# ferreiraluisa/implementation-phd-lab-vision

Hardware: AMD Instinct MI355X
Metric: H36M frames/sec ResNet-50 feature extraction (higher is better)
Workload: dtype bf16; 1 GPU; ResNet-50[:-1] bf16 forward, batch 256 x 224x224x3 fp32 NCHW frames per GPU (BASELINE configs[1]), seeded synthetic weights, (N,2048) fp32 features; batch_per_gpu=256, micro_batch=0, lanes=2, lanes_requested=2, lanes_mode=2 lanes (1.092 x one lane), input=f32, parallelism=frames sharded over 1 rank(s)

## Files before the change

### implementation_phd_lab_vision_amd/csrc/kernels.h

```cpp
#pragma once
#include <hip/hip_runtime.h>
#include <stdint.h>
#include <type_traits>

typedef __attribute__((ext_vector_type(8))) __bf16 bf16x8;
typedef __attribute__((ext_vector_type(4))) float f32x4;
typedef __attribute__((ext_vector_type(4))) unsigned int u32x4;
typedef __attribute__((ext_vector_type(2))) unsigned int u32x2;

#define GLOBAL_AS __attribute__((address_space(1)))
#define LDS_AS __attribute__((address_space(3)))

__device__ __forceinline__ float bf16_bits_to_f32(unsigned int hi16) { return __uint_as_float(hi16 << 16); }

__device__ __forceinline__ unsigned int pack_bf16x2(float lo, float hi) {
    typedef __attribute__((ext_vector_type(2))) __bf16 bf16x2;
    typedef __attribute__((ext_vector_type(2))) float f32x2;
    f32x2 v = {lo, hi};
    bf16x2 b = __builtin_convertvector(v, bf16x2);
    return __builtin_bit_cast(unsigned int, b);
}

typedef __attribute__((ext_vector_type(8))) _Float16 f16x8;
typedef __attribute__((ext_vector_type(2))) _Float16 f16x2;

template <int ET>
__device__ __forceinline__ f32x4 mfma_e(bf16x8 a, bf16x8 b, f32x4 c) {
    if constexpr (ET == 0) return __builtin_amdgcn_mfma_f32_16x16x32_bf16(a, b, c, 0, 0, 0);
    else return __builtin_amdgcn_mfma_f32_16x16x32_f16(__builtin_bit_cast(f16x8, a), __builtin_bit_cast(f16x8, b), c, 0, 0, 0);
}
typedef __attribute__((ext_vector_type(16))) float f32x16;
template <int ET>
__device__ __forceinline__ f32x16 mfma32_e(bf16x8 a, bf16x8 b, f32x16 c) {
    if constexpr (ET == 0) return __builtin_amdgcn_mfma_f32_32x32x16_bf16(a, b, c, 0, 0, 0);
    else return __builtin_amdgcn_mfma_f32_32x32x16_f16(__builtin_bit_cast(f16x8, a), __builtin_bit_cast(f16x8, b), c, 0, 0, 0);
}
typedef __attribute__((ext_vector_type(8))) int i32x8;
__device__ __forceinline__ f32x4 mfma_fp8_k128(bf16x8 a0, bf16x8 a1, bf16x8 b0, bf16x8 b1, f32x4 c) {
    const u32x4 al = __builtin_bit_cast(u32x4, a0), ah = __builtin_bit_cast(u32x4, a1);
    const u32x4 bl = __builtin_bit_cast(u32x4, b0), bh = __builtin_bit_cast(u32x4, b1);
    const i32x8 a = {(int)al[0], (int)al[1], (int)al[2], (int)al[3], (int)ah[0], (int)ah[1], (int)ah[2], (int)ah[3]};
    const i32x8 b = {(int)bl[0], (int)bl[1], (int)bl[2], (int)bl[3], (int)bh[0], (int)bh[1], (int)bh[2], (int)bh[3]};
    return __builtin_amdgcn_mfma_scale_f32_16x16x128_f8f6f4(a, b, c, 0, 0, 0, 0x7f7f7f7f, 0, 0x7f7f7f7f);
}
__device__ __forceinline__ unsigned pack4_fp8(float v0, float v1, float v2, float v3) {
    v0 = __builtin_amdgcn_fmed3f(v0, -448.0f, 448.0f); v1 = __builtin_amdgcn_fmed3f(v1, -448.0f, 448.0f);
    v2 = __builtin_amdgcn_fmed3f(v2, -448.0f, 448.0f); v3 = __builtin_amdgcn_fmed3f(v3, -448.0f, 448.0f);
    int w = __builtin_amdgcn_cvt_pk_fp8_f32(v0, v1, 0, false);
    w = __builtin_amdgcn_cvt_pk_fp8_f32(v2, v3, w, true);
    return (unsigned)w;
}
template <int ET>
__device__ __forceinline__ unsigned int pack2_e(float lo, float hi) {
    if constexpr (ET == 0) {
        return pack_bf16x2(lo, hi);
    } else {
        lo = __builtin_amdgcn_fmed3f(lo, -65504.0f, 65504.0f);
        hi = __builtin_amdgcn_fmed3f(hi, -65504.0f, 65504.0f);
        const f16x2 b = {(_Float16)lo, (_Float16)hi};
        return __builtin_bit_cast(unsigned int, b);
    }
}
template <int ET>
__device__ __forceinline__ float unpack_lo_e(unsigned int u) {
    if constexpr (ET == 0) return bf16_bits_to_f32(u & 0xffffu);
    else return (float)__builtin_bit_cast(f16x2, u)[0];
}
template <int ET>
__device__ __forceinline__ float unpack_hi_e(unsigned int u) {
    if constexpr (ET == 0) return __uint_as_float(u & 0xffff0000u);
    else return (float)__builtin_bit_cast(f16x2, u)[1];
}

struct FastDiv {
    unsigned mul, shr;
};

struct ConvArgs {
    const __bf16* x;
    const __bf16* w;
    const float* bias;
    const __bf16* res;
    __bf16* y;
    int N, H, W, Cin, Ho, Wo, Cout;
    int ks, stride, pad, relu;
    int M;
    int HoWo;
    int cin_chunks;
    int nk;
    int Ktot;
    int n_ctiles;
    int n_blocks;
    int x_back;
    unsigned x_records;
    unsigned w_bytes;
    unsigned y_bytes;
    FastDiv div_howo, div_wo, div_ctiles;
    int x_cstride;
    int x_wrap;
    int y_cstride;
    int et;
    float oscale, rscale;
    float q_inv;
    const __bf16* x2;
    int H2, W2, stride2, x2_cstride, cc1;
    unsigned x2_records;
#if defined(R50_STAMP)
    unsigned long long* dbg;
#endif
};

#if defined(R50_STAMP)
#define R50_STAMP_DECL unsigned long long st_prev = __builtin_readcyclecounter(), st_sum[8] = {0, 0, 0, 0, 0, 0, 0, 0}; const unsigned long long st_rt0 = __builtin_amdgcn_s_memrealtime();
#define R50_MARK(i) { __builtin_amdgcn_sched_barrier(0); const unsigned long long st_now = __builtin_readcyclecounter(); st_sum[i] += st_now - st_prev; st_prev = st_now; __builtin_amdgcn_sched_barrier(0); }
#define R50_STAMP_FLUSH(nw) st_sum[7] = __builtin_amdgcn_s_memrealtime() - st_rt0;    \
    if (a.dbg && (threadIdx.x & 63) == 0) { _Pragma("unroll") for (int q = 0; q < 8; ++q) \
        a.dbg[((size_t)blockIdx.x * (nw) + (threadIdx.x >> 6)) * 8 + q] = st_sum[q]; }
#else
#define R50_STAMP_DECL
#define R50_MARK(i)
#define R50_STAMP_FLUSH(nw)
#endif

__device__ __forceinline__ unsigned fast_div(unsigned n, FastDiv d) {
    return d.mul == 0u ? n : (__umulhi(n, d.mul) >> d.shr);
}

#ifndef XCD_REMAP
#define XCD_REMAP 1
#endif
__device__ __forceinline__ int xcd_remap(int bid, int nblk) {
    const int q = nblk >> 3, r = nblk & 7, xcd = bid & 7;
    const int base = (xcd < r) ? xcd * (q + 1) : r * (q + 1) + (xcd - r) * q;
    return base + (bid >> 3);
}

template <int LO, int HI>
__device__ __forceinline__ void wait_vmcnt_range(int n) {
    if constexpr (LO == HI) {
        asm volatile("s_waitcnt vmcnt(%0)" ::"n"(LO) : "memory");
    } else {
        constexpr int MID = (LO + HI) / 2;
        if (n <= MID) wait_vmcnt_range<LO, MID>(n);
        else wait_vmcnt_range<MID + 1, HI>(n);
    }
}
__device__ __forceinline__ void wait_vmcnt(int n) { wait_vmcnt_range<0, 63>(n < 0 ? 0 : (n > 63 ? 63 : n)); }

__device__ __forceinline__ unsigned relu_bf16x2(unsigned v) {
    typedef __attribute__((ext_vector_type(2))) short s16x2;
    const s16x2 z = {0, 0};
    return __builtin_bit_cast(unsigned, __builtin_elementwise_max(__builtin_bit_cast(s16x2, v), z));
}

constexpr unsigned kOobOffset = 0x80000000u;

template <int ET, int BC, int BP, int WC, int WP, int NSTAGE, bool SPLIT = false>
__global__ __launch_bounds__(WC * WP * 64) void igemm_bf16_kernel(const ConvArgs a) {
#if defined(__HIP_DEVICE_COMPILE__)
    constexpr int NT = WC * WP * 64;
    constexpr int MR = BC / WC / 16;
    constexpr int NR = BP / WP / 16;
    static_assert(MR >= 2 && (MR % 2) == 0, "wave needs >= 32 couts");
    static_assert(NSTAGE == 2 || NSTAGE == 3, "2 or 3 LDS stages");
    constexpr int RPP = NT / 8;
    static_assert(BC % RPP == 0 && BP % (16 * WP) == 0, "cout rows fill whole staging passes; pixels come in 16-blocks per wave");
    constexpr int WROWS = BC / RPP;
    constexpr int XROWS = (BP + RPP - 1) / RPP;
    constexpr int BP_PAD = XROWS * RPP;
    constexpr int PASS_BYTES = NT * 16;
    constexpr int STAGE_BYTES = (BC + BP_PAD) * 128;
    constexpr int LOADS_PER_STAGE = WROWS + XROWS;
    constexpr int D = NSTAGE - 1;

    extern __shared__ __attribute__((aligned(16))) char smem[];

    const int tid = threadIdx.x;
    const int lane = tid & 63;
    const int wave = __builtin_amdgcn_readfirstlane(tid >> 6);
    const int wave_c = wave / WP, wave_p = wave % WP;
    const int fr = lane & 15, fq = lane >> 4;
    const int srow = tid >> 3;
    const int slot = tid & 7;
    const int lchunk = slot ^ (srow & 7);

    const int grid = gridDim.x;
    const int first = xcd_remap(blockIdx.x, grid);
    const int my_tiles = (a.n_blocks - first + grid - 1) / grid;
    const int total = my_tiles * a.nk;

    const __amdgpu_buffer_rsrc_t rsrc_w =
        __builtin_amdgcn_make_buffer_rsrc(const_cast<__bf16*>(a.w), 0, a.w_bytes, 0x00020000);
    const __amdgpu_buffer_rsrc_t rsrc_x = __builtin_amdgcn_make_buffer_rsrc(
        const_cast<char*>(reinterpret_cast<const char*>(a.x) - a.x_back), 0, a.x_records, 0x00020000);
    const __amdgpu_buffer_rsrc_t rsrc_y = __builtin_amdgcn_make_buffer_rsrc(a.y, 0, a.y_bytes, 0x00020000);
    const __amdgpu_buffer_rsrc_t rsrc_r =
        __builtin_amdgcn_make_buffer_rsrc(const_cast<__bf16*>(a.res), 0, a.res ? a.y_bytes : 0u, 0x00020000);

    unsigned x_voff[XROWS], x_mask[XROWS], w_voff[WROWS];
    auto decode_tile = [&](int tile) {
        const int pt = (int)fast_div((unsigned)tile, a.div_ctiles);
        const int ct = tile - pt * a.n_ctiles;
        const int c0 = ct * BC, p0 = pt * BP;
#pragma unroll
        for (int i = 0; i < XROWS; ++i) {
            const int m = p0 + i * RPP + srow;
            unsigned mask = 0u, voff = kOobOffset;
            if ((BP_PAD == BP || i * RPP + srow < BP) && m < a.M) {
                const int n = (int)fast_div((unsigned)m, a.div_howo);
                const int r = m - n * a.HoWo;
                const int ho = (int)fast_div((unsigned)r, a.div_wo);
                const int wo = r - ho * a.Wo;
                const int hc = ho * a.stride, wc = wo * a.stride;
                voff = (unsigned)(((n * a.H + hc) * a.W + wc) * a.x_cstride + lchunk * 8) * 2u;
                if (a.ks == 1) {
                    mask = 1u;
                } else {
                    const unsigned hm = (hc >= a.pad ? 1u : 0u) | 2u | (hc - a.pad + 2 < a.H ? 4u : 0u);
                    const unsigned wm = (wc >= a.pad ? 1u : 0u) | 2u | (wc - a.pad + 2 < a.W ? 4u : 0u);
                    mask = ((hm & 1u) ? wm : 0u) | ((hm & 2u) ? (wm << 3) : 0u) | ((hm & 4u) ? (wm << 6) : 0u);
                }
            }
            x_voff[i] = voff;
            x_mask[i] = mask;
        }
#pragma unroll
        for (int i = 0; i < WROWS; ++i) {
            const int rho = i * RPP + srow;
            const int cl = (rho & ~31) | (rho & 3) | (((rho >> 4) & 1) << 2) | (((rho >> 2) & 3) << 3);
            w_voff[i] = (unsigned)((c0 + cl) * a.Ktot + lchunk * 8) * 2u;
        }
    };
    int i_tile = first, i_k = 0, i_tap = 0, i_cc = 0, i_dw = 0, i_wofs = 0, i_tapofs = 0, i_buf = 0;
    const int row_adv = (a.W - a.ks) * a.x_cstride * 2;
    decode_tile(i_tile);
    auto stage_issue = [&]() {
        char* sbase = smem + i_buf * STAGE_BYTES;
        const int xcc = (i_cc >= a.x_wrap) ? i_cc - a.x_wrap : i_cc;
        const int xofs = __builtin_amdgcn_readfirstlane(i_tapofs + xcc * 128);
        const int wofs = __builtin_amdgcn_readfirstlane(i_wofs);
        const int tap = __builtin_amdgcn_readfirstlane(i_tap);
#pragma unroll
        for (int i = 0; i < WROWS; ++i)
            __builtin_amdgcn_raw_ptr_buffer_load_lds(rsrc_w, (LDS_AS void*)(sbase + i * PASS_BYTES + wave * 1024), 16,
                                                     w_voff[i], wofs, 0, 0);
#pragma unroll
        for (int i = 0; i < XROWS; ++i) {
            const unsigned voff = ((x_mask[i] >> tap) & 1u) ? x_voff[i] : kOobOffset;
            __builtin_amdgcn_raw_ptr_buffer_load_lds(rsrc_x, (LDS_AS void*)(sbase + BC * 128 + i * PASS_BYTES + wave * 1024),
                                                     16, voff, xofs, 0, 0);
        }
        i_buf = (i_buf == NSTAGE - 1) ? 0 : i_buf + 1;
        i_wofs += 128;
        if (++i_cc == a.cin_chunks) {
            i_cc = 0;
            ++i_tap;
            i_tapofs += a.x_cstride * 2;
            if (++i_dw == a.ks) { i_dw = 0; i_tapofs += row_adv; }
        }
        if (++i_k == a.nk) {
            i_k = 0; i_tap = 0; i_cc = 0; i_dw = 0; i_wofs = 0; i_tapofs = 0;
            i_tile += grid;
            if (i_tile < a.n_blocks) decode_tile(i_tile);
        }
    };

    f32x4 acc[MR][NR];
    constexpr bool BIG = (MR * NR > 16);
    constexpr bool LEAN = (NT >= 1024);
    constexpr bool PREFETCH_RES = !SPLIT && !BIG && !LEAN;
    u32x4 res_reg[PREFETCH_RES ? MR / 2 : 1][PREFETCH_RES ? NR : 1];
    const bool has_res = (a.res != nullptr);
    const int fphys0 = (fq ^ (fr & 7)) << 4;
    const int w_frag = (wave_c * MR * 16 + fr) * 128;
    const int x_frag = BC * 128 + (wave_p * NR * 16 + fr) * 128;
    const int cout_lane = wave_c * MR * 16 + 8 * fq;
    const int pix_lane = wave_p * NR * 16 + fr;
    int c_tile = first, c_k = 0, c_buf = 0;
    unsigned y_voff = 0u;
    const unsigned y_rowstep = (unsigned)(16 * a.y_cstride * 2);

    auto tile_begin = [&]() {
        const int pt = (int)fast_div((unsigned)c_tile, a.div_ctiles);
// ... 2106 lines not shown
                const int prow = (32 * k + srow) % ROWS;
                const int lchunk = (lt & 7) ^ (prow & 7);
                const unsigned p = (unsigned)(p0 + prow);
                const unsigned n = p / HOWO, r = p - n * HOWO, ho = r / OW, wo = r - ho * OW;
                const unsigned q = a.x_sub ? p : (n * WI + 2 * ho) * WI + 2 * wo;
                const bool ok = prow < limit;
                vt[k] = ok ? (p * CT2 + lchunk * 8) * 2u : kOobOffset;
                vx[k] = ok ? (q * CX + lchunk * 8) * 2u : kOobOffset;
            }
        };
        auto issue_x = [&](auto grp_c) {
            constexpr int GRP = decltype(grp_c)::value;
#pragma unroll
            for (int i = 7 * GRP; i < 7 * GRP + 7; ++i) {
                const int sl = __builtin_amdgcn_readfirstlane((32 * i + 8 * w) / ROWS);
                char* dst = smem + XR + i * 4096 + w * 1024;
                if (GRP == 0) __builtin_amdgcn_raw_ptr_buffer_load_lds(rs_t2, (LDS_AS void*)dst, 16, vt[i % 7], sl * 128, 0, 0);
                else __builtin_amdgcn_raw_ptr_buffer_load_lds(rs_x, (LDS_AS void*)dst, 16, vx[i % 7], (sl - 2) * 128, 0, 0);
            }
        };
        using G0 = std::integral_constant<int, 0>;
        using G1 = std::integral_constant<int, 1>;
        using G2 = std::integral_constant<int, 2>;
        f32x4 accB[2][NR];
        unsigned rvo[OC_PASSES];
        auto out_rows = [&](int tile) {
            const int p0 = tile * a.bp;
            const int limit = (a.M - p0 < a.bp) ? a.M - p0 : a.bp;
#pragma unroll
            for (int i = 0; i < OC_PASSES; ++i) {
                const int R = 32 * i + srow;
                const int sl = R / ROWS, prow = R - ROWS * sl;
                const int lchunk = (lt & 7) ^ (prow & 7);
                rvo[i] = (prow < limit) ? (unsigned)((p0 + prow) * COUT + sl * 64 + lchunk * 8) * 2u : kOobOffset;
            }
        };
        auto y1n_store = [&](int tile) {
            const int p0 = tile * a.bp;
            const int limit = (a.M - p0 < a.bp) ? a.M - p0 : a.bp;
#pragma unroll
            for (int j = 0; j < NR; ++j) {
                const f32x4 lo = accB[0][j], hi = accB[1][j];
                u32x4 o = (u32x4){pack2_e<ET>(lo[0], lo[1]), pack2_e<ET>(lo[2], lo[3]), pack2_e<ET>(hi[0], hi[1]), pack2_e<ET>(hi[2], hi[3])};
#pragma unroll
                for (int e = 0; e < 4; ++e) o[e] = relu_bf16x2(o[e]);
                const unsigned voff = (16 * j + fr < limit) ? (unsigned)((p0 + 16 * j + fr) * C1N + 32 * w + 8 * fq) * 2u : kOobOffset;
                __builtin_amdgcn_raw_buffer_store_b128(o, rs_y1, voff, 0, 0);
            }
        };
        auto init_accb = [&]() {
            const f32x4 lo = *reinterpret_cast<const f32x4*>(smem + B1_OFF + (32 * w + 8 * fq) * 4);
            const f32x4 hi = *reinterpret_cast<const f32x4*>(smem + B1_OFF + (32 * w + 8 * fq + 4) * 4);
#pragma unroll
            for (int j = 0; j < NR; ++j) { accB[0][j] = lo; accB[1][j] = hi; }
        };
        x_rows(first);
        issue_x(G0{}); issue_x(G1{}); issue_x(G2{});
        w_load_half(sofs_of(0, 6), wA, 0); w_load_half(sofs_of(0, 6), wA, 1);
        w_load_half(sofs_of(0, 7), wB, 0); w_load_half(sofs_of(0, 7), wB, 1);
        asm volatile("s_waitcnt vmcnt(0) lgkmcnt(0)" ::: "memory");
        __builtin_amdgcn_s_barrier();
        init_accb();
        __builtin_amdgcn_s_barrier();
        unsigned tl = 0;
        R50_STAMP_DECL
        for (int tile = first; tile < a.n_tiles; tile += grid, ++tl) {
            out_rows(tile);
            for (int c = 0; c < NCH; ++c) {
                const char* xb = smem + OUTC + (c & 1) * 2 * SLOT;
                if (c == NCH - 2) x_rows(tile + grid);
                w_step(sofs_of(c + 1, 6), wA, xb, accB[0], accB[1]);
                R50_MARK(2)
                if (c == NCH - 2) { spin_until(0, 4u * (tl + 1)); issue_x(G0{}); }
                R50_MARK(5)
                if (c == NCH - 1) {
                    asm volatile("s_waitcnt vmcnt(4)" ::: "memory");
                    signal(3);
                }
                R50_MARK(6)
                w_step(sofs_of(c + 1, 7), wB, xb + SLOT, accB[0], accB[1]);
                R50_MARK(2)
                if (c == NCH - 2) { spin_until(1, 4u * (tl + 1)); issue_x(G1{}); }
                R50_MARK(5)
#if defined(R50_STAMP)
                __builtin_amdgcn_sched_barrier(0);
                asm volatile("s_nop 0" ::"v"(accB[1][NR - 1]), "v"(accB[0][NR - 1]) : "memory");
#endif
                R50_MARK(2)
                __builtin_amdgcn_sched_barrier(0);
                {
                    const int cofs = __builtin_amdgcn_readfirstlane(c * 256);
                    u32x4 v[OC_PASSES];
#pragma unroll
                    for (int i = 0; i < OC_PASSES; ++i) v[i] = *reinterpret_cast<const u32x4*>(xb + i * 4096 + lt * 16);
#pragma unroll
                    for (int i = 0; i < OC_PASSES; ++i)
                        __builtin_amdgcn_raw_buffer_store_b128(v[i], rs_out, rvo[i], cofs, 0);
                }
                asm volatile("s_waitcnt lgkmcnt(0)" ::: "memory");
                R50_MARK(3)
                if (c == NCH - 2) {
                    spin_until(2, 4u * (tl + 1));
                    issue_x(G2{});
                    R50_MARK(5)
                    asm volatile("s_waitcnt vmcnt(14)" ::: "memory");
                    R50_MARK(6)
                }
                if (c == NCH - 1) { y1n_store(tile); init_accb(); }
                R50_MARK(0)
                __builtin_amdgcn_s_barrier();
                R50_MARK(4)
            }
        }
        R50_STAMP_FLUSH(8)
    }
#else
    (void)a;
#endif
}

struct Block2Args {
    const __bf16* t1;
    const __bf16* w2;
    const float* b2;
    const __bf16* w3;
    const float* b3;
    const __bf16* res;
    __bf16* out;
    const __bf16* w1;
    const float* b1;
    __bf16* y1n;
    int N;
    int n_tiles;
};

#define B2_LOADER_LOOP _Pragma("unroll")
template <int ET, int C1N>
__global__ __launch_bounds__(768) void bneck_block2_kernel(const Block2Args a) {
#if defined(__HIP_DEVICE_COMPILE__)
    static_assert(C1N == 0 || C1N == 128, "next conv1: none or 512 -> 128");
    constexpr int IW = 28, TR = 7, PW = 32, PP = (TR + 2) * PW;
    constexpr int XPASS = (PP + 31) / 32, XBUF = XPASS * 32 * 128;
    constexpr int NPX = TR * IW;
    constexpr int SLOT = 208 * 128;
    constexpr int XB_OFF = 0, T2_OFF = C1N ? 0 : 2 * SLOT, OUTC_OFF = 2 * SLOT, RESB_OFF = 3 * SLOT, RESB_BYTES = 224 * 128;
    constexpr int RING_OFF = C1N ? RESB_OFF + RESB_BYTES : 4 * SLOT;
    constexpr int NST = 3, WSTAGE = 128 * 128, WPASS = 4;
    constexpr int BIAS_OFF = RING_OFF + NST * WSTAGE;
    constexpr int NCONV = 18, SPT = NCONV + (C1N ? 16 : 8);
    static_assert(2 * XBUF <= (C1N ? RESB_OFF : RING_OFF) && BIAS_OFF + 768 * 4 <= 163840, "LDS map");
    extern __shared__ __attribute__((aligned(16))) char smem[];
    const int tid = threadIdx.x, lane = tid & 63;
    const int wave = __builtin_amdgcn_readfirstlane(tid >> 6);
    const int grid = gridDim.x, first = blockIdx.x;

    {
        float v;
        if (tid < 128) v = a.b2[tid];
        else if (tid < 640) v = a.b3[tid - 128];
        else v = (C1N ? a.b1[tid - 640] : 0.f);
        reinterpret_cast<float*>(smem + BIAS_OFF)[tid] = v;
    }

    if (wave >= 8) {
        const int lw = wave - 8, lt = tid - 512;
        const int srow = lt >> 3, slot = lt & 7;
        const __amdgpu_buffer_rsrc_t rs_w2 = __builtin_amdgcn_make_buffer_rsrc(const_cast<__bf16*>(a.w2), 0, 128u * 1152u * 2u, 0x00020000);
        const __amdgpu_buffer_rsrc_t rs_w3 = __builtin_amdgcn_make_buffer_rsrc(const_cast<__bf16*>(a.w3), 0, 512u * 128u * 2u, 0x00020000);
        const __amdgpu_buffer_rsrc_t rs_w1 = __builtin_amdgcn_make_buffer_rsrc(const_cast<__bf16*>(a.w1), 0, C1N ? 128u * 512u * 2u : 0u, 0x00020000);
        const __amdgpu_buffer_rsrc_t rs_x = __builtin_amdgcn_make_buffer_rsrc(const_cast<__bf16*>(a.t1), 0, (unsigned)a.N * (784u * 256u), 0x00020000);
        const __amdgpu_buffer_rsrc_t rs_res = __builtin_amdgcn_make_buffer_rsrc(const_cast<__bf16*>(a.res), 0, (unsigned)a.N * (784u * 1024u), 0x00020000);
        const __amdgpu_buffer_rsrc_t rs_out = __builtin_amdgcn_make_buffer_rsrc(a.out, 0, (unsigned)a.N * (784u * 1024u), 0x00020000);
        unsigned w2v[WPASS], w3v[WPASS], w1v[WPASS], x_voff[XPASS];
#pragma unroll
        for (int i = 0; i < WPASS; ++i) {
            const int rho = i * 32 + srow;
            const int cl = (rho & ~31) | (rho & 3) | (((rho >> 4) & 1) << 2) | (((rho >> 2) & 3) << 3);
            const unsigned ch = (unsigned)((slot ^ (rho & 7)) * 8);
            w2v[i] = ((unsigned)cl * 1152u + ch) * 2u;
            w1v[i] = ((unsigned)cl * 512u + ch) * 2u;
            if (C1N) {
                const int rp = rho & 63, ks = rho >> 6;
                const int cl2 = (rp & ~31) | (rp & 3) | (((rp >> 4) & 1) << 2) | (((rp >> 2) & 3) << 3);
                w3v[i] = ((unsigned)cl2 * 128u + (unsigned)ks * 64u + ch) * 2u;
            } else {
                w3v[i] = ((unsigned)cl * 128u + ch) * 2u;
            }
        }
        auto decode_band = [&](int tile) {
            const int n = tile >> 2, band = tile & 3;
#pragma unroll
            for (int i = 0; i < XPASS; ++i) {
                const int q = i * 32 + srow;
                const int rr = q / PW, cc = q - rr * PW;
                const int y = band * TR + rr - 1, x = cc - 1;
                const bool ok = q < PP && tile < a.n_tiles && (unsigned)y < 28u && (unsigned)x < 28u;
                x_voff[i] = (ok) ? (unsigned)(((n * 28 + y) * 28 + x) * 128 + (slot ^ (cc & 7)) * 8) * 2u : kOobOffset;
            }
        };
        auto issue_band = [&](int c2) {
            const int xofs = __builtin_amdgcn_readfirstlane(c2 * 128);
#pragma unroll
            for (int i = 0; i < XPASS; ++i)
                __builtin_amdgcn_raw_ptr_buffer_load_lds(rs_x, (LDS_AS void*)(smem + XB_OFF + c2 * XBUF + i * 4096 + lw * 1024), 16, x_voff[i], xofs, 0, 0);
        };
        unsigned rv[7];
#pragma unroll
        for (int i = 0; i < 7; ++i) {
            const int R = 32 * i + srow;
            rv[i] = (R < NPX) ? ((unsigned)R * 512u + (unsigned)((slot ^ (R & 7)) * 8)) * 2u : kOobOffset;
        }
        auto issue_res = [&](unsigned tile_pix0, int c) {
            const int sofs = __builtin_amdgcn_readfirstlane((int)(tile_pix0 * 1024u) + c * 128);
#pragma unroll
            for (int i = 0; i < 7; ++i)
                __builtin_amdgcn_raw_ptr_buffer_load_lds(rs_res, (LDS_AS void*)(smem + RESB_OFF + i * 4096 + lw * 1024), 16, rv[i], sofs, 0, 0);
        };
        auto copy_out = [&](unsigned tile_pix0, int c) {
            const int sofs = __builtin_amdgcn_readfirstlane((int)(tile_pix0 * 1024u) + c * 128);
            u32x4 v[7];
#pragma unroll
            for (int i = 0; i < 7; ++i) v[i] = *reinterpret_cast<const u32x4*>(smem + OUTC_OFF + i * 4096 + lt * 16);
#pragma unroll
            for (int i = 0; i < 7; ++i) __builtin_amdgcn_raw_buffer_store_b128(v[i], rs_out, rv[i], sofs, 0);
        };
        int ring = 0;
        auto stage_issue = [&](int p) {
            char* sbase = smem + RING_OFF + ring * WSTAGE + lw * 1024;
            ring = (ring == NST - 1) ? 0 : ring + 1;
            if (p < NCONV) {
                const int c2 = p >= 9 ? 1 : 0, tap = p - 9 * c2;
                const int sofs = __builtin_amdgcn_readfirstlane((tap * 128 + c2 * 64) * 2);
#pragma unroll
                for (int i = 0; i < WPASS; ++i)
                    __builtin_amdgcn_raw_ptr_buffer_load_lds(rs_w2, (LDS_AS void*)(sbase + i * 4096), 16, w2v[i], sofs, 0, 0);
            } else {
                const int q = p - NCONV, c = q >> 1, r = q & 1;
                if (!C1N || r == 0) {
                    const int sofs = __builtin_amdgcn_readfirstlane(C1N ? c * 64 * 128 * 2 : (c * 128 * 128 + r * 64) * 2);
#pragma unroll
                    for (int i = 0; i < WPASS; ++i)
                        __builtin_amdgcn_raw_ptr_buffer_load_lds(rs_w3, (LDS_AS void*)(sbase + i * 4096), 16, w3v[i], sofs, 0, 0);
                } else {
                    const int sofs = __builtin_amdgcn_readfirstlane(c * 64 * 2);
#pragma unroll
                    for (int i = 0; i < WPASS; ++i)
                        __builtin_amdgcn_raw_ptr_buffer_load_lds(rs_w1, (LDS_AS void*)(sbase + i * 4096), 16, w1v[i], sofs, 0, 0);
                }
            }
        };
        auto wait_younger = [&](int n) { wait_vmcnt(n); };
        decode_band(first);
        issue_band(0);
        issue_band(1);
        stage_issue(0);
        stage_issue(1);
        asm volatile("s_waitcnt vmcnt(4) lgkmcnt(0)" ::: "memory");
        __builtin_amdgcn_s_barrier();
        bool first_tile = true;
        int carry = 0;
        constexpr int PBAND = C1N ? SPT - 1 : SPT - 2;
#pragma unroll 1
        for (int tile = first; tile < a.n_tiles; tile += grid) {
            const bool has_next = tile + grid < a.n_tiles;
            const unsigned tile_pix0 = (unsigned)((tile >> 2) * 784 + (tile & 3) * NPX);
            B2_LOADER_LOOP
            for (int p = 0; p < SPT; ++p) {
                if (p == NCONV || (C1N && p > NCONV && ((p - NCONV) & 1) == 1)) __builtin_amdgcn_s_barrier();
                int younger = carry;
                carry = 0;
                if (p == 0 && !first_tile) { issue_band(1); younger += XPASS; }
                if (p == PBAND && has_next) { decode_band(tile + grid); issue_band(0); if (C1N) younger = 0; else younger += XPASS; }
                const bool bpos = C1N && p > NCONV && ((p - NCONV) & 1) == 1;
                if (C1N && p == NCONV - 2) { issue_res(tile_pix0, 0); younger += 7; }
                if (bpos && p + 1 < SPT) { issue_res(tile_pix0, (p - NCONV + 1) / 2); younger += 7; }
                const bool st = (p + 2 < SPT) || has_next;
                if (st) { stage_issue(p + 2 < SPT ? p + 2 : p + 2 - SPT); younger += WPASS; }
                const bool cpos = C1N && p > NCONV + 1 && (((p - NCONV) & 1) == 0 || p == SPT - 1);
                if (cpos) {
                    copy_out(tile_pix0, p == SPT - 1 ? 7 : (p - NCONV) / 2 - 1);
                    younger += 7;
                    carry = 7;
                }
                wait_younger(younger);
                __builtin_amdgcn_s_barrier();
            }
            first_tile = false;
        }
    } else {
        const int wave_c = wave & 3, wave_p = wave >> 2;
        const int wave_a = wave & 1, wave_q = wave >> 1;
        const int qb0 = wave_q == 0 ? 0 : 1 + 3 * wave_q;
        const int fr = lane & 15, fq = lane >> 4;
        const __amdgpu_buffer_rsrc_t rs_res = __builtin_amdgcn_make_buffer_rsrc(const_cast<__bf16*>(a.res), 0, (unsigned)a.N * (784u * 1024u), 0x00020000);
        const __amdgpu_buffer_rsrc_t rs_out = __builtin_amdgcn_make_buffer_rsrc(a.out, 0, (unsigned)a.N * (784u * 1024u), 0x00020000);
        const __amdgpu_buffer_rsrc_t rs_y1 = __builtin_amdgcn_make_buffer_rsrc(a.y1n, 0, (unsigned)a.N * (784u * 256u), 0x00020000);
        const int w_row = (wave_c * 32 + fr) * 128;
        const int w_rowa = (wave_a * 32 + fr) * 128;
        const int w_ph0 = (fq ^ (fr & 7)) << 4;
        const int ch_lane = wave_c * 32 + 8 * fq;
        const int cha_lane = wave_a * 32 + 8 * fq;
        const int p0 = 16 * 7 * wave_p + fr, pb0 = p0 * 128 + ((fq ^ (p0 & 7)) << 4);
        const int pa0 = 16 * qb0 + fr, pba0 = pa0 * 128 + ((fq ^ (pa0 & 7)) << 4);
        const int cf_x = (wave_c & 1) << 6, cf_a = (wave_c >> 1) * SLOT;

        auto run = [&](auto nrw_c, auto nq_c) {
            constexpr int NRW = decltype(nrw_c)::value, NQ = decltype(nq_c)::value;
// ... 45 lines not shown
#pragma unroll 1
            for (int tile = first; tile < a.n_tiles; tile += grid) {
                const unsigned tile_pix0 = (unsigned)((tile >> 2) * 784 + (tile & 3) * NPX);
                {
                    const f32x4 lo = *reinterpret_cast<const f32x4*>(smem + BIAS_OFF + (ch_lane) * 4);
                    const f32x4 hi = *reinterpret_cast<const f32x4*>(smem + BIAS_OFF + (ch_lane + 4) * 4);
#pragma unroll
                    for (int j = 0; j < 7; ++j) { accC[0][j] = lo; accC[1][j] = hi; }
                }
                int opq = 0;
                asm volatile("" : "+v"(opq));
                {
                    int vb[3][2];
#pragma unroll
                    for (int kw = 0; kw < 3; ++kw)
#pragma unroll
                        for (int kk = 0; kk < 2; ++kk) vb[kw][kk] = (fr + kw + opq) * 128 + (((fq + 4 * kk) ^ ((fr + kw) & 7)) << 4);
#pragma unroll 1
                    for (int c2 = 0; c2 < 2; ++c2) {
                        const char* const xc = smem + XB_OFF + c2 * XBUF + 7 * 2048 * wave_p;
#pragma unroll
                        for (int tap = 0; tap < 9; ++tap) {
                            const int kh = tap / 3, kw = tap - 3 * kh;
                            const char* const x0 = xc + vb[kw][0] + kh * (PW * 128);
                            const char* const x1 = xc + vb[kw][1] + kh * (PW * 128);
                            gemm64(std::integral_constant<int, 7>{}, smem + RING_OFF + cbuf * WSTAGE + w_row, [&](int t) {
                                return (t >= 7 ? x1 : x0) + (t % 7) * 2048;
                            }, accC);
                            stage_done();
                        }
                    }
                }
#pragma unroll
                for (int j = 0; j < 7; ++j) {
                    const int b = 7 * wave_p + j;
                    const int col = 16 * (b & 1) + fr, p = 28 * (b >> 1) + col + opq;
                    if (col < IW) *reinterpret_cast<u32x4*>(smem + T2_OFF + cf_a + ((p * 128 + ((fq ^ (p & 7)) << 4)) ^ cf_x)) = pack_relu(accC[0][j], accC[1][j]);
                }
                if constexpr (C1N != 0) {
                    const f32x4 lo = *reinterpret_cast<const f32x4*>(smem + BIAS_OFF + (640 + ch_lane) * 4);
                    const f32x4 hi = *reinterpret_cast<const f32x4*>(smem + BIAS_OFF + (640 + ch_lane + 4) * 4);
#pragma unroll
                    for (int j = 0; j < NRW; ++j) { acc[0][j] = lo; acc[1][j] = hi; }
                }
                asm volatile("s_waitcnt lgkmcnt(0)" ::: "memory");
                __builtin_amdgcn_s_barrier();
                if constexpr (C1N == 0) {
                    const unsigned pix0 = tile_pix0 + (unsigned)p0;
#pragma unroll 1
                    for (int c = 0; c < 4; ++c) {
                        u32x4 r[NRW];
#pragma unroll
                        for (int j = 0; j < NRW; ++j) {
                            const unsigned voff = (p0 + 16 * j < NPX) ? ((pix0 + 16 * j) * 512u + (unsigned)(c * 128 + ch_lane)) * 2u : kOobOffset;
                            r[j] = __builtin_amdgcn_raw_buffer_load_b128(rs_res, voff, 0, 0);
                        }
                        {
                            const f32x4 lo = *reinterpret_cast<const f32x4*>(smem + BIAS_OFF + (128 + c * 128 + ch_lane) * 4);
                            const f32x4 hi = *reinterpret_cast<const f32x4*>(smem + BIAS_OFF + (128 + c * 128 + ch_lane + 4) * 4);
#pragma unroll
                            for (int j = 0; j < NRW; ++j) { acc[0][j] = lo; acc[1][j] = hi; }
                        }
#pragma unroll 1
                        for (int ks = 0; ks < 2; ++ks) {
                            const char* bb = smem + T2_OFF + ks * SLOT;
                            gemm64(NRWc, smem + RING_OFF + cbuf * WSTAGE + w_row, [&](int t) { return bb + ((pb0 + 2048 * (t % NRW)) ^ (t >= NRW ? 64 : 0)); }, acc);
                            stage_done();
                        }
#pragma unroll
                        for (int j = 0; j < NRW; ++j) {
                            f32x4 lo = acc[0][j], hi = acc[1][j];
                            add_identity(lo, hi, r[j]);
                            const u32x4 o = pack_relu(lo, hi);
                            const unsigned voff = (p0 + 16 * j < NPX) ? ((pix0 + 16 * j) * 512u + (unsigned)(c * 128 + ch_lane)) * 2u : kOobOffset;
                            __builtin_amdgcn_raw_buffer_store_b128(o, rs_out, voff, 0, 0);
                        }
                    }
                } else {
#pragma unroll 1
                    for (int c = 0; c < 8; ++c) {
                        {
                            const f32x4 lo = *reinterpret_cast<const f32x4*>(smem + BIAS_OFF + (128 + c * 64 + cha_lane) * 4);
                            const f32x4 hi = *reinterpret_cast<const f32x4*>(smem + BIAS_OFF + (128 + c * 64 + cha_lane + 4) * 4);
#pragma unroll
                            for (int j = 0; j < NQ; ++j) { accA[0][j] = lo; accA[1][j] = hi; }
                        }
#pragma unroll
                        for (int ks = 0; ks < 2; ++ks) {
                            const char* bb = smem + T2_OFF + ks * SLOT;
                            gemm64(NQc, smem + RING_OFF + cbuf * WSTAGE + ks * 8192 + w_rowa, [&](int t) { return bb + ((pba0 + 2048 * (t % NQ)) ^ (t >= NQ ? 64 : 0)); }, accA);
                        }
                        stage_done();
                        {
                            u32x4 r[NQ];
#pragma unroll
                            for (int j = 0; j < NQ; ++j) r[j] = *reinterpret_cast<const u32x4*>(smem + RESB_OFF + ((pba0 + 2048 * j) ^ (wave_a << 6)));
#pragma unroll
                            for (int j = 0; j < NQ; ++j) {
                                f32x4 lo = accA[0][j], hi = accA[1][j];
                                add_identity(lo, hi, r[j]);
                                *reinterpret_cast<u32x4*>(smem + OUTC_OFF + ((pba0 + 2048 * j) ^ (wave_a << 6))) = pack_relu(lo, hi);
                            }
                        }
                        asm volatile("s_waitcnt lgkmcnt(0)" ::: "memory");
                        __builtin_amdgcn_s_barrier();
                        {
                            const char* bb = smem + OUTC_OFF;
                            gemm64(NRWc, smem + RING_OFF + cbuf * WSTAGE + w_row, [&](int t) { return bb + ((pb0 + 2048 * (t % NRW)) ^ (t >= NRW ? 64 : 0)); }, acc);
                            stage_done();
                        }
                    }
                    const unsigned pix0 = tile_pix0 + (unsigned)p0;
#pragma unroll
                    for (int j = 0; j < NRW; ++j) {
                        const u32x4 o = pack_relu(acc[0][j], acc[1][j]);
                        const unsigned voff = (p0 + 16 * j < NPX) ? ((pix0 + 16 * j) * 128u + (unsigned)ch_lane) * 2u : kOobOffset;
                        __builtin_amdgcn_raw_buffer_store_b128(o, rs_y1, voff, 0, 0);
                    }
                }
            }
        };
        asm volatile("s_waitcnt lgkmcnt(0)" ::: "memory");
        __builtin_amdgcn_s_barrier();
        if (wave_p == 0) {
            if (wave_q == 0) run(std::integral_constant<int, 7>{}, std::integral_constant<int, 4>{});
            else run(std::integral_constant<int, 7>{}, std::integral_constant<int, 3>{});
        } else {
            run(std::integral_constant<int, 6>{}, std::integral_constant<int, 3>{});
        }
    }
#else
    (void)a;
#endif
}

struct Block1Args {
    const __bf16* t1;
    const __bf16* w2;
    const float* b2;
    const __bf16* w3;
    const float* b3;
    const __bf16* res;
    const __bf16* wd;
    const float* bd;
    __bf16* out;
    const __bf16* w1;
    const float* b1;
    __bf16* y1n;
    int N;
    int n_tiles;
    int out_sub;
};

template <int ET, int C1N, bool DS = false>
__global__ __launch_bounds__(768) void bneck_block1_kernel(const Block1Args a) {
#if defined(__HIP_DEVICE_COMPILE__)
    static_assert(C1N == 64 || C1N == 128, "next conv1: 256 -> 64 or 256 -> 128");
    constexpr int IW = 56, TR = 4, PW = IW + 2, PP = (TR + 2) * PW;
    constexpr int XPASS = (PP + 31) / 32, XBUF = XPASS * 32 * 128;
    constexpr int NPX = TR * IW;
    constexpr int SLOT = NPX * 128;
    constexpr int XB_OFF = 0, T2_OFF = XBUF, OUTC_OFF = T2_OFF + SLOT, RESB_OFF = OUTC_OFF + SLOT, RING_OFF = RESB_OFF + SLOT;
    constexpr int NST = 3, WSTAGE = 64 * 128, WPASS = 2;
    constexpr int BIAS_OFF = RING_OFF + NST * WSTAGE;
    constexpr int NB1 = C1N / 64;
    constexpr int NA = DS ? 2 : 1;
    constexpr int NCONV = 9, LCH = NA + NB1, SPT = NCONV + 4 * LCH;
    constexpr int BD_IDX = 64 + 256 + C1N;
    static_assert(BIAS_OFF + (448 + 256) * 4 <= 163840, "LDS map");
    extern __shared__ __attribute__((aligned(16))) char smem[];
    const int tid = threadIdx.x, lane = tid & 63;
    const int wave = __builtin_amdgcn_readfirstlane(tid >> 6);
    const int grid = gridDim.x, first = blockIdx.x;

    if (tid < 64 + 256 + C1N) {
        float v;
        if (tid < 64) v = a.b2[tid];
        else if (tid < 320) v = a.b3[tid - 64];
        else v = a.b1[tid - 320];
        reinterpret_cast<float*>(smem + BIAS_OFF)[tid] = v;
    }
    if (DS && tid >= 512) reinterpret_cast<float*>(smem + BIAS_OFF)[BD_IDX + tid - 512] = a.bd[tid - 512];

    if (wave >= 8) {
        const int lw = wave - 8, lt = tid - 512;
        const int srow = lt >> 3, slot = lt & 7;
        const __amdgpu_buffer_rsrc_t rs_w2 = __builtin_amdgcn_make_buffer_rsrc(const_cast<__bf16*>(a.w2), 0, 64u * 576u * 2u, 0x00020000);
        const __amdgpu_buffer_rsrc_t rs_w3 = __builtin_amdgcn_make_buffer_rsrc(const_cast<__bf16*>(a.w3), 0, 256u * 64u * 2u, 0x00020000);
        const __amdgpu_buffer_rsrc_t rs_w1 = __builtin_amdgcn_make_buffer_rsrc(const_cast<__bf16*>(a.w1), 0, (unsigned)C1N * 256u * 2u, 0x00020000);
        const __amdgpu_buffer_rsrc_t rs_x = __builtin_amdgcn_make_buffer_rsrc(const_cast<__bf16*>(a.t1), 0, (unsigned)a.N * (3136u * 128u), 0x00020000);
        const __amdgpu_buffer_rsrc_t rs_res = __builtin_amdgcn_make_buffer_rsrc(const_cast<__bf16*>(a.res), 0, (unsigned)a.N * (3136u * (DS ? 128u : 512u)), 0x00020000);
        const __amdgpu_buffer_rsrc_t rs_wd = __builtin_amdgcn_make_buffer_rsrc(const_cast<__bf16*>(DS ? a.wd : a.w3), 0, 256u * 64u * 2u, 0x00020000);
        const __amdgpu_buffer_rsrc_t rs_out = __builtin_amdgcn_make_buffer_rsrc(a.out, 0, (unsigned)a.N * (3136u * 512u), 0x00020000);
        unsigned w2v[WPASS], w3v[WPASS], w1v[WPASS], x_voff[XPASS], rv[7], rvx[7], rvs[7];
#pragma unroll
        for (int i = 0; i < WPASS; ++i) {
            const int rho = i * 32 + srow;
            const int cl = (rho & ~31) | (rho & 3) | (((rho >> 4) & 1) << 2) | (((rho >> 2) & 3) << 3);
            const unsigned ch = (unsigned)((slot ^ (rho & 7)) * 8);
            w2v[i] = ((unsigned)cl * 576u + ch) * 2u;
            w3v[i] = ((unsigned)cl * 64u + ch) * 2u;
            w1v[i] = ((unsigned)cl * 256u + ch) * 2u;
        }
#pragma unroll
        for (int i = 0; i < 7; ++i) {
            const int R = 32 * i + srow;
            rv[i] = ((unsigned)R * 256u + (unsigned)((slot ^ (R & 7)) * 8)) * 2u;
            rvx[i] = ((unsigned)R * 64u + (unsigned)((slot ^ (R & 7)) * 8)) * 2u;
            const int sr = R / 56, sc = R - 56 * sr;
            rvs[i] = (a.out_sub && !((sr | sc) & 1)) ? ((unsigned)((sr >> 1) * 28 + (sc >> 1)) * 256u + (unsigned)((slot ^ (R & 7)) * 8)) * 2u : kOobOffset;
        }
        auto decode_band = [&](int tile) {
            const int n = tile / 14, tr = tile - n * 14;
#pragma unroll
            for (int i = 0; i < XPASS; ++i) {
                const int q = i * 32 + srow;
                const int rr = q / PW, cc = q - rr * PW;
                const int y = tr * TR + rr - 1, x = cc - 1;
                const bool ok = q < PP && tile < a.n_tiles && (unsigned)y < 56u && (unsigned)x < 56u;
                x_voff[i] = ok ? (unsigned)(((n * 56 + y) * 56 + x) * 64 + (slot ^ ((rr * IW + cc) & 7)) * 8) * 2u : kOobOffset;
            }
        };
        auto issue_band = [&](int i0, int i1) {
#pragma unroll
            for (int i = 0; i < XPASS; ++i)
                if (i >= i0 && i < i1)
                    __builtin_amdgcn_raw_ptr_buffer_load_lds(rs_x, (LDS_AS void*)(smem + XB_OFF + i * 4096 + lw * 1024), 16, x_voff[i], 0, 0, 0);
        };
        auto issue_res = [&](unsigned tile_pix0, int c) {
            const int sofs = __builtin_amdgcn_readfirstlane(DS ? (int)(tile_pix0 * 128u) : (int)(tile_pix0 * 512u) + c * 128);
#pragma unroll
            for (int i = 0; i < 7; ++i)
                __builtin_amdgcn_raw_ptr_buffer_load_lds(rs_res, (LDS_AS void*)(smem + RESB_OFF + i * 4096 + lw * 1024), 16, DS ? rvx[i] : rv[i], sofs, 0, 0);
        };
        auto copy_out = [&](unsigned tile_pix0, int c) {
            const int sofs = __builtin_amdgcn_readfirstlane((int)((a.out_sub ? tile_pix0 >> 2 : tile_pix0) * 512u) + c * 128);
            u32x4 v[7];
#pragma unroll
            for (int i = 0; i < 7; ++i) v[i] = *reinterpret_cast<const u32x4*>(smem + OUTC_OFF + i * 4096 + lt * 16);
#pragma unroll
            for (int i = 0; i < 7; ++i) __builtin_amdgcn_raw_buffer_store_b128(v[i], rs_out, a.out_sub ? rvs[i] : rv[i], sofs, 0);
        };
        int ring = 0;
        auto stage_issue = [&](int p) {
            char* sbase = smem + RING_OFF + ring * WSTAGE + lw * 1024;
            ring = (ring == NST - 1) ? 0 : ring + 1;
            if (p < NCONV) {
                const int sofs = __builtin_amdgcn_readfirstlane(p * 64 * 2);
#pragma unroll
                for (int i = 0; i < WPASS; ++i)
                    __builtin_amdgcn_raw_ptr_buffer_load_lds(rs_w2, (LDS_AS void*)(sbase + i * 4096), 16, w2v[i], sofs, 0, 0);
            } else {
                const int q = p - NCONV, c = q / LCH, r = q - c * LCH;
                if (r < NA) {
                    const int sofs = __builtin_amdgcn_readfirstlane(c * 64 * 64 * 2);
#pragma unroll
                    for (int i = 0; i < WPASS; ++i)
                        __builtin_amdgcn_raw_ptr_buffer_load_lds(r == 0 ? rs_w3 : rs_wd, (LDS_AS void*)(sbase + i * 4096), 16, w3v[i], sofs, 0, 0);
                } else {
                    const int sofs = __builtin_amdgcn_readfirstlane(((r - NA) * 64 * 256 + c * 64) * 2);
#pragma unroll
                    for (int i = 0; i < WPASS; ++i)
                        __builtin_amdgcn_raw_ptr_buffer_load_lds(rs_w1, (LDS_AS void*)(sbase + i * 4096), 16, w1v[i], sofs, 0, 0);
                }
            }
        };
        auto wait_younger = [&](int n) { wait_vmcnt(n); };
        decode_band(first);
        issue_band(0, XPASS);
        stage_issue(0);
        stage_issue(1);
        asm volatile("s_waitcnt vmcnt(2) lgkmcnt(0)" ::: "memory");
        __builtin_amdgcn_s_barrier();
        int carry = 0;
#pragma unroll 1
        for (int tile = first; tile < a.n_tiles; tile += grid) {
            const bool has_next = tile + grid < a.n_tiles;
            const unsigned tile_pix0 = (unsigned)((tile / 14) * 3136 + (tile % 14) * NPX);
            B2_LOADER_LOOP
            for (int p = 0; p < SPT; ++p) {
                const int q = p - NCONV, c = q >= 0 ? q / LCH : -1, r = q >= 0 ? q - c * LCH : -1;
                if (p == NCONV || r == NA) __builtin_amdgcn_s_barrier();
                int younger = carry;
                carry = 0;
                if (p == NCONV - 2) { issue_res(tile_pix0, 0); younger += 7; }
                if (!DS && r == 1 && c < 3) { issue_res(tile_pix0, c + 1); younger += 7; }
                if (has_next && p >= NCONV && p < NCONV + 4) {
                    if (p == NCONV) decode_band(tile + grid);
                    const int i0 = 3 * (p - NCONV), i1 = (p == NCONV + 3) ? XPASS : i0 + 3;
                    issue_band(i0, i1);
                    younger += i1 - i0;
                }
                const bool st = (p + 2 < SPT) || has_next;
                if (st) { stage_issue(p + 2 < SPT ? p + 2 : p + 2 - SPT); younger += WPASS; }
                const bool cpos = (C1N == 64) ? ((r == 0 && c >= 1) || p == SPT - 1) : (r == NA + 1);
                if (cpos) {
                    copy_out(tile_pix0, (C1N == 64 && p != SPT - 1) ? c - 1 : c);
                    younger += 7;
                    carry = 7;
                }
                wait_younger(younger);
                __builtin_amdgcn_s_barrier();
            }
        }
    } else {
        const int wave_a = wave & 1, wave_q = wave >> 1;
        const int qb0 = wave_q < 2 ? 4 * wave_q : 8 + 3 * (wave_q - 2);
        const int fr = lane & 15, fq = lane >> 4;
        const __amdgpu_buffer_rsrc_t rs_y1 = __builtin_amdgcn_make_buffer_rsrc(a.y1n, 0, (unsigned)a.N * (3136u * C1N * 2u), 0x00020000);
        const int w_row = (wave_a * 32 + fr) * 128;
        const int w_ph0 = (fq ^ (fr & 7)) << 4;
        const int ch_lane = wave_a * 32 + 8 * fq;
        const int p0 = 16 * qb0 + fr, pb0 = p0 * 128 + ((fq ^ (p0 & 7)) << 4), cf_x = wave_a << 6;

        auto run = [&](auto nq_c) {
            constexpr int NQ = decltype(nq_c)::value;
            f32x4 acc[2][NQ], accB[NB1][2][NQ], accD[2][DS ? NQ : 1];
            int cbuf = 0;
            auto gemm64 = [&](const char* wb, auto xaddr, auto& ac) {
                constexpr int NS = 2 * NQ, PD = 3;
                bf16x8 x[NS], wf[2], wg[2];
#pragma unroll
                for (int m = 0; m < 2; ++m) wf[m] = *reinterpret_cast<const bf16x8*>(wb + m * 2048 + w_ph0);
#pragma unroll
                for (int m = 0; m < 2; ++m) wg[m] = *reinterpret_cast<const bf16x8*>(wb + m * 2048 + (w_ph0 ^ 64));
#pragma unroll
                for (int t = 0; t < PD; ++t) x[t] = *reinterpret_cast<const bf16x8*>(xaddr(t));
#pragma unroll
                for (int t = 0; t < NS; ++t) {
#pragma unroll
                    for (int m = 0; m < 2; ++m) ac[m][t % NQ] = mfma_e<ET>(t >= NQ ? wg[m] : wf[m], x[t], ac[m][t % NQ]);
                    if (t + PD < NS) x[t + PD] = *reinterpret_cast<const bf16x8*>(xaddr(t + PD));
                }
                __builtin_amdgcn_sched_group_barrier(0x100, 4 + PD, 0);
#pragma unroll
                for (int t = 0; t < NS; ++t) {
                    __builtin_amdgcn_sched_group_barrier(0x008, 2, 0);
                    if (t + PD < NS) __builtin_amdgcn_sched_group_barrier(0x100, 1, 0);
                }
                __builtin_amdgcn_sched_barrier(0);
            };
            auto stage_done = [&]() {
                cbuf = (cbuf == NST - 1) ? 0 : cbuf + 1;
                __builtin_amdgcn_s_barrier();
            };
            auto pack_relu = [&](const f32x4& lo, const f32x4& hi) {
                u32x4 o = (u32x4){pack2_e<ET>(lo[0], lo[1]), pack2_e<ET>(lo[2], lo[3]), pack2_e<ET>(hi[0], hi[1]), pack2_e<ET>(hi[2], hi[3])};
#pragma unroll
                for (int e = 0; e < 4; ++e) o[e] = relu_bf16x2(o[e]);
                return o;
            };
            auto set_bias = [&](f32x4 (&ac)[2][NQ], int fidx) {
                const f32x4 lo = *reinterpret_cast<const f32x4*>(smem + BIAS_OFF + (fidx + ch_lane) * 4);
                const f32x4 hi = *reinterpret_cast<const f32x4*>(smem + BIAS_OFF + (fidx + ch_lane + 4) * 4);
#pragma unroll
                for (int j = 0; j < NQ; ++j) { ac[0][j] = lo; ac[1][j] = hi; }
            };
#pragma unroll 1
            for (int tile = first; tile < a.n_tiles; tile += grid) {
                const unsigned pix0 = (unsigned)((tile / 14) * 3136 + (tile % 14) * NPX + p0);
                set_bias(acc, 0);
                {
                    int opq = 0;
                    asm volatile("" : "+v"(opq));
                    int q0[NQ];
#pragma unroll
                    for (int j = 0; j < NQ; ++j) {
                        const int p = p0 + 16 * j + opq;
                        const int r = p / IW, c = p - r * IW;
                        q0[j] = r * PW + c;
                    }
#pragma unroll 1
                    for (int tap = 0; tap < 9; ++tap) {
                        const int kh = (tap >= 6) ? 2 : (tap >= 3) ? 1 : 0, kw = tap - 3 * kh;
                        const int sw = (kh * PW + kw) * 128 + ((fq ^ ((p0 + kh * IW + kw) & 7)) << 4);
                        gemm64(smem + RING_OFF + cbuf * WSTAGE + w_row, [&](int t) {
                            return smem + XB_OFF + q0[t % NQ] * 128 + (t >= NQ ? (sw ^ 64) : sw);
                        }, acc);
                        stage_done();
                    }
                }
#pragma unroll
                for (int j = 0; j < NQ; ++j) *reinterpret_cast<u32x4*>(smem + T2_OFF + ((pb0 + 2048 * j) ^ cf_x)) = pack_relu(acc[0][j], acc[1][j]);
#pragma unroll
                for (int h = 0; h < NB1; ++h) set_bias(accB[h], 320 + 64 * h);
                asm volatile("s_waitcnt lgkmcnt(0)" ::: "memory");
                __builtin_amdgcn_s_barrier();
#pragma unroll 1
                for (int c = 0; c < 4; ++c) {
                    set_bias(acc, 64 + 64 * c);
                    gemm64(smem + RING_OFF + cbuf * WSTAGE + w_row, [&](int t) { return smem + T2_OFF + ((pb0 + 2048 * (t % NQ)) ^ (t >= NQ ? 64 : 0)); }, acc);
                    stage_done();
                    if constexpr (DS) {
                        set_bias(accD, BD_IDX + 64 * c);
                        gemm64(smem + RING_OFF + cbuf * WSTAGE + w_row, [&](int t) { return smem + RESB_OFF + ((pb0 + 2048 * (t % NQ)) ^ (t >= NQ ? 64 : 0)); }, accD);
                        stage_done();
                    }
                    {
                        u32x4 rr[NQ];
#pragma unroll
                        for (int j = 0; j < NQ; ++j) {
                            if constexpr (DS) rr[j] = (u32x4){pack2_e<ET>(accD[0][j][0], accD[0][j][1]), pack2_e<ET>(accD[0][j][2], accD[0][j][3]),
                                                              pack2_e<ET>(accD[1][j][0], accD[1][j][1]), pack2_e<ET>(accD[1][j][2], accD[1][j][3])};
                            else rr[j] = *reinterpret_cast<const u32x4*>(smem + RESB_OFF + ((pb0 + 2048 * j) ^ cf_x));
                        }
#pragma unroll
                        for (int j = 0; j < NQ; ++j) {
                            f32x4 lo = acc[0][j], hi = acc[1][j];
                            lo[0] += unpack_lo_e<ET>(rr[j][0]); lo[1] += unpack_hi_e<ET>(rr[j][0]);
                            lo[2] += unpack_lo_e<ET>(rr[j][1]); lo[3] += unpack_hi_e<ET>(rr[j][1]);
                            hi[0] += unpack_lo_e<ET>(rr[j][2]); hi[1] += unpack_hi_e<ET>(rr[j][2]);
                            hi[2] += unpack_lo_e<ET>(rr[j][3]); hi[3] += unpack_hi_e<ET>(rr[j][3]);
                            *reinterpret_cast<u32x4*>(smem + OUTC_OFF + ((pb0 + 2048 * j) ^ cf_x)) = pack_relu(lo, hi);
                        }
                    }
                    asm volatile("s_waitcnt lgkmcnt(0)" ::: "memory");
                    __builtin_amdgcn_s_barrier();
#pragma unroll
                    for (int h = 0; h < NB1; ++h) {
                        gemm64(smem + RING_OFF + cbuf * WSTAGE + w_row, [&](int t) { return smem + OUTC_OFF + ((pb0 + 2048 * (t % NQ)) ^ (t >= NQ ? 64 : 0)); }, accB[h]);
                        stage_done();
                    }
                }
#pragma unroll
                for (int h = 0; h < NB1; ++h)
#pragma unroll
                    for (int j = 0; j < NQ; ++j) {
                        const u32x4 o = pack_relu(accB[h][0][j], accB[h][1][j]);
                        __builtin_amdgcn_raw_buffer_store_b128(o, rs_y1, ((pix0 + 16 * j) * (unsigned)C1N + (unsigned)(64 * h + ch_lane)) * 2u, 0, 0);
                    }
            }
        };
        asm volatile("s_waitcnt lgkmcnt(0)" ::: "memory");
        __builtin_amdgcn_s_barrier();
        if (wave_q < 2) run(std::integral_constant<int, 4>{});
        else run(std::integral_constant<int, 3>{});
    }
#else
    (void)a;
#endif
}

struct ResizeArgs {
    const unsigned char* src;
    unsigned char* dst;
    int T, H, W, top, left, hh, ww, out;
    int px, py;
    int float_mode;
    int hflip, trev;
};

__device__ __forceinline__ void resize_taps(int i, int in_size, int out_size, int prec, bool float_mode, int& i0, int& w0, int& w1) {
    if (float_mode) {
// ... 2917 lines not shown
```

Measured before the change: 102,900 frames/s.

## Keep part of block1 weight stages resident in loader registers; remap tiles across XCDs

In the block1 bottleneck kernel, the loader waves now preload a configurable number of weight stages (by default 8 for the C1N=64 non-downsample variant) into registers once per block. They write those stages into the LDS ring from registers on each tile instead of reissuing global buffer-to-LDS loads, which cuts repeated weight fetch traffic and vmcnt waits. XCD-aware block remapping is also enabled by default for that same variant, so consecutive tiles land on the same XCD for L2 locality. The cost is extra VGPR pressure in the loader waves and added LDS write plus lgkmcnt waits, and the wait count bookkeeping in the pipeline changes.

```diff
diff --git a/implementation_phd_lab_vision_amd/csrc/kernels.h b/implementation_phd_lab_vision_amd/csrc/kernels.h
--- a/implementation_phd_lab_vision_amd/csrc/kernels.h
+++ b/implementation_phd_lab_vision_amd/csrc/kernels.h
@@ -129,6 +129,10 @@
 #ifndef XCD_REMAP
 #define XCD_REMAP 1
 #endif
+#ifndef BODY_XCD_REMAP
+#define BODY_XCD_REMAP -1
+#endif
+#define BODY_XCD_REMAP_ON(dflt) (BODY_XCD_REMAP >= 0 ? BODY_XCD_REMAP != 0 : (dflt))
 __device__ __forceinline__ int xcd_remap(int bid, int nblk) {
     const int q = nblk >> 3, r = nblk & 7, xcd = bid & 7;
     const int base = (xcd < r) ? xcd * (q + 1) : r * (q + 1) + (xcd - r) * q;
@@ -2541,7 +2545,7 @@
     extern __shared__ __attribute__((aligned(16))) char smem[];
     const int tid = threadIdx.x, lane = tid & 63;
     const int wave = __builtin_amdgcn_readfirstlane(tid >> 6);
-    const int grid = gridDim.x, first = blockIdx.x;
+    const int grid = gridDim.x, first = BODY_XCD_REMAP_ON(false) ? xcd_remap(blockIdx.x, grid) : (int)blockIdx.x;
 
     {
         float v;
@@ -2893,6 +2897,18 @@
     int out_sub;
 };
 
+#ifndef B1_RESIDENT_W
+#define B1_RESIDENT_W -1
+#endif
+#ifndef B1_RESIDENT_C64
+#define B1_RESIDENT_C64 8
+#endif
+#ifndef B1_RESIDENT_C128
+#define B1_RESIDENT_C128 0
+#endif
+#ifndef B1_RESIDENT_DS
+#define B1_RESIDENT_DS 0
+#endif
 template <int ET, int C1N, bool DS = false>
 __global__ __launch_bounds__(768) void bneck_block1_kernel(const Block1Args a) {
 #if defined(__HIP_DEVICE_COMPILE__)
@@ -2908,11 +2924,12 @@
     constexpr int NA = DS ? 2 : 1;
     constexpr int NCONV = 9, LCH = NA + NB1, SPT = NCONV + 4 * LCH;
     constexpr int BD_IDX = 64 + 256 + C1N;
+    constexpr int NRES = B1_RESIDENT_W >= 0 ? (B1_RESIDENT_W < SPT ? B1_RESIDENT_W : SPT) : (DS ? B1_RESIDENT_DS : C1N == 128 ? B1_RESIDENT_C128 : B1_RESIDENT_C64);
     static_assert(BIAS_OFF + (448 + 256) * 4 <= 163840, "LDS map");
     extern __shared__ __attribute__((aligned(16))) char smem[];
     const int tid = threadIdx.x, lane = tid & 63;
     const int wave = __builtin_amdgcn_readfirstlane(tid >> 6);
-    const int grid = gridDim.x, first = blockIdx.x;
+    const int grid = gridDim.x, first = BODY_XCD_REMAP_ON(C1N == 64 && !DS) ? xcd_remap(blockIdx.x, grid) : (int)blockIdx.x;
 
     if (tid < 64 + 256 + C1N) {
         float v;
@@ -2983,35 +3000,53 @@
             for (int i = 0; i < 7; ++i) __builtin_amdgcn_raw_buffer_store_b128(v[i], rs_out, a.out_sub ? rvs[i] : rv[i], sofs, 0);
         };
         int ring = 0;
+        auto stage_src = [&](int p, auto f) {
+            if (p < NCONV) {
+                f(rs_w2, w2v, __builtin_amdgcn_readfirstlane(p * 64 * 2));
+            } else {
+                const int q = p - NCONV, c = q / LCH, r = q - c * LCH;
+                if (r < NA)
+                    f(r == 0 ? rs_w3 : rs_wd, w3v, __builtin_amdgcn_readfirstlane(c * 64 * 64 * 2));
+                else
+                    f(rs_w1, w1v, __builtin_amdgcn_readfirstlane(((r - NA) * 64 * 256 + c * 64) * 2));
+            }
+        };
         auto stage_issue = [&](int p) {
             char* sbase = smem + RING_OFF + ring * WSTAGE + lw * 1024;
             ring = (ring == NST - 1) ? 0 : ring + 1;
-            if (p < NCONV) {
-                const int sofs = __builtin_amdgcn_readfirstlane(p * 64 * 2);
+            stage_src(p, [&](const __amdgpu_buffer_rsrc_t rs, const unsigned (&wv)[WPASS], int sofs) {
 #pragma unroll
                 for (int i = 0; i < WPASS; ++i)
-                    __builtin_amdgcn_raw_ptr_buffer_load_lds(rs_w2, (LDS_AS void*)(sbase + i * 4096), 16, w2v[i], sofs, 0, 0);
-            } else {
-                const int q = p - NCONV, c = q / LCH, r = q - c * LCH;
-                if (r < NA) {
-                    const int sofs = __builtin_amdgcn_readfirstlane(c * 64 * 64 * 2);
-#pragma unroll
-                    for (int i = 0; i < WPASS; ++i)
-                        __builtin_amdgcn_raw_ptr_buffer_load_lds(r == 0 ? rs_w3 : rs_wd, (LDS_AS void*)(sbase + i * 4096), 16, w3v[i], sofs, 0, 0);
-                } else {
-                    const int sofs = __builtin_amdgcn_readfirstlane(((r - NA) * 64 * 256 + c * 64) * 2);
-#pragma unroll
-                    for (int i = 0; i < WPASS; ++i)
-                        __builtin_amdgcn_raw_ptr_buffer_load_lds(rs_w1, (LDS_AS void*)(sbase + i * 4096), 16, w1v[i], sofs, 0, 0);
-                }
-            }
+                    __builtin_amdgcn_raw_ptr_buffer_load_lds(rs, (LDS_AS void*)(sbase + i * 4096), 16, wv[i], sofs, 0, 0);
+            });
+        };
+        auto res_slot = [](int p) { return p >= NCONV ? p - NCONV : SPT - NCONV + p; };
+        u32x4 wres[NRES > 0 ? NRES : 1][WPASS];
+#pragma unroll
+        for (int p = 0; p < SPT; ++p)
+            if (res_slot(p) < NRES)
+                stage_src(p, [&](const __amdgpu_buffer_rsrc_t rs, const unsigned (&wv)[WPASS], int sofs) {
+#pragma unroll
+                    for (int i = 0; i < WPASS; ++i) wres[res_slot(p)][i] = __builtin_amdgcn_raw_buffer_load_b128(rs, wv[i], sofs, 0);
+                });
+        auto stage_write = [&](int p) {
+            char* sbase = smem + RING_OFF + ring * WSTAGE + lw * 1024 + lane * 16;
+            ring = (ring == NST - 1) ? 0 : ring + 1;
+#pragma unroll
+            for (int i = 0; i < WPASS; ++i) *reinterpret_cast<u32x4*>(sbase + i * 4096) = wres[res_slot(p)][i];
+        };
+        auto stage_put = [&](int p) {
+            if (res_slot(p) < NRES) { stage_write(p); return 0; }
+            stage_issue(p);
+            return WPASS;
         };
         auto wait_younger = [&](int n) { wait_vmcnt(n); };
         decode_band(first);
         issue_band(0, XPASS);
-        stage_issue(0);
-        stage_issue(1);
-        asm volatile("s_waitcnt vmcnt(2) lgkmcnt(0)" ::: "memory");
+        stage_put(0);
+        constexpr int PRO1 = (SPT - NCONV + 1 < NRES) ? 0 : WPASS;
+        stage_put(1);
+        asm volatile("s_waitcnt vmcnt(%0) lgkmcnt(0)" ::"n"(PRO1) : "memory");
         __builtin_amdgcn_s_barrier();
         int carry = 0;
 #pragma unroll 1
@@ -3033,13 +3068,15 @@
                     younger += i1 - i0;
                 }
                 const bool st = (p + 2 < SPT) || has_next;
-                if (st) { stage_issue(p + 2 < SPT ? p + 2 : p + 2 - SPT); younger += WPASS; }
+                const int ps = p + 2 < SPT ? p + 2 : p + 2 - SPT;
+                if (st) younger += stage_put(ps);
                 const bool cpos = (C1N == 64) ? ((r == 0 && c >= 1) || p == SPT - 1) : (r == NA + 1);
                 if (cpos) {
                     copy_out(tile_pix0, (C1N == 64 && p != SPT - 1) ? c - 1 : c);
                     younger += 7;
                     carry = 7;
                 }
+                if (st && res_slot(ps) < NRES) asm volatile("s_waitcnt lgkmcnt(0)" ::: "memory");
                 wait_younger(younger);
                 __builtin_amdgcn_s_barrier();
             }
```

Result: no change. 103,900 frames/s (median of 6 runs) (+0.9%).
